# seagochen/unet-segment-pytorch

Hardware: NVIDIA B200
Metric: AttentionUNet 512^2 train images/sec (whole job; per GPU = value / n_gpus) (higher is better)
Workload: dtype bf16

## Files before the change

include/unetb200.h:

```cpp
#ifndef UNETB200_H
#define UNETB200_H
#include <stddef.h>
#include <stdint.h>

#ifdef __cplusplus
extern "C" {
#endif

#define UB2_OK 0
#define UB2_ERR_SHAPE (-1)
#define UB2_ERR_ALIGN (-2)
#define UB2_ERR_WORKSPACE (-3)
#define UB2_ERR_DRIVER (-4)
#define UB2_ERR_ARCH (-5)

int ub2_version(void);
int ub2_num_sms(void);
int ub2_set_conv_mode(int mode);
int ub2_last_conv_variant(void);


int ub2_conv_fwd(const void* in0, int ld_in0, int C0, const void* in1, int ld_in1, int C1,
                 const void* wgt, void* out0, int ld0, void* out1, int ld1, int split, int N, int H,
                 int W, int Cout, int taps, const float* scale, const float* shift, int relu,
                 int accumulate, double* stats, int stats_rows, int* stats_rows_used,
                 int bn_override, int grid_override, void* stream);

int ub2_conv_wgrad(const void* in0, int ld_in0, int C0, const void* in1, int ld_in1, int C1,
                   const void* dy, int ld_dy, float* partial, int max_splits, int* splits_used,
                   int N, int H, int W, int Cout, int taps, int splits_override, void* stream);

int ub2_wgrad_reduce(float* partial, int splits, int Cout, int Cin, int taps, float* grad,
                     int accumulate, void* stream);

#define UB2_REDUCE_MAX_ITEMS 32
typedef struct Ub2ReduceItem {
  float* partial;
  float* grad;
  int splits, Cout, Cin, taps;
} Ub2ReduceItem;
int ub2_wgrad_reduce_multi(const Ub2ReduceItem* items, int n, int accumulate, void* stream);

int ub2_pack_conv_weight(const float* w, void* fwd, void* dgrad, int Cout, int Cin, int taps,
                         const float* out_scale, void* stream);
int ub2_pack_conv_weights_multi(const long long* desc, const int* blocks, int nblocks, void* stream);


int ub2_bn_finalize(const double* partials, int rows, int C, double count, const float* gamma,
                    const float* beta, float* running_mean, float* running_var, long long* nbt,
                    float momentum, float eps, float* scale, float* shift, float* mean, float* invstd,
                    void* stream);
int ub2_bn_eval_coeffs(const float* gamma, const float* beta, const float* running_mean,
                       const float* running_var, float eps, int C, float* scale, float* shift,
                       void* stream);
int ub2_bn_act(const void* y, int ld_y, const float* scale, const float* shift, void* a, int ld_a,
               void* pooled, int ld_p, unsigned char* pidx, int N, int H, int W, int C, int relu,
               void* stream);
int ub2_bn_bwd_rows(int N, int H, int W, int C, int pool);
int ub2_bn_bwd_reduce(const void* dA, int ld_da, const void* dP, int ld_dp, const unsigned char* pidx,
                      const void* y, int ld_y, const float* scale, const float* shift, double* partials,
                      int rows, int N, int H, int W, int C, int relu, void* stream);
int ub2_bn_bwd_finalize(const double* partials, int rows, int C, double count, const float* gamma,
                        const float* mean, const float* invstd, int frozen, float* dgamma, float* dbeta,
                        float* coef, void* stream);
int ub2_bn_bwd_apply(const void* dA, int ld_da, const void* dP, int ld_dp, const unsigned char* pidx,
                     const void* y, int ld_y, const float* scale, const float* shift, const float* coef,
                     void* dY, int ld_dy, int N, int H, int W, int C, int relu, void* stream);


int ub2_upsample_fwd(const void* in, int ld_in, void* out, int ld_out, int N, int hin, int win, int hu,
                     int wu, int Ho, int Wo, int C, void* stream);
int ub2_upsample_bwd(const void* dout, int ld_dout, void* din, int ld_din, int accumulate, int N,
                     int hin, int win, int hu, int wu, int Ho, int Wo, int C, void* stream);

int ub2_shuffle2x2_fwd(const void* t, int ld_t, void* out, int ld_out, int N, int h, int w, int C, int Ho, int Wo,
                       void* stream);
int ub2_shuffle2x2_rows(int N, int h, int w, int C, int Ho, int Wo);
int ub2_shuffle2x2_bwd(const void* dout, int ld_dout, void* dt, int ld_dt, double* partials, int rows, float* dbias,
                       int N, int h, int w, int C, int Ho, int Wo, void* stream);
int ub2_pack_convt_weight(const float* w, const float* bias, void* fwd, void* dg, float* scale4, float* shift4,
                          int Cin, int Cout, void* stream);
int ub2_convt_wgrad_reduce(const float* partial, int splits, int Cin, int Cout, float* grad, int accumulate,
                           void* stream);
int ub2_resize_planes_fwd(const float* in, float* out, int planes, int hin, int win, int Ho, int Wo, void* stream);
int ub2_resize_planes_bwd(const float* dout, float* din, int planes, int hin, int win, int Ho, int Wo,
                          void* stream);


int ub2_gate_rows(int N, int H, int W, int C);
int ub2_gate_strip_rows(int N, int H, int W, int C);
int ub2_gate_upstats(const void* q, int ld_q, int N, int hin, int win, int H, int W, int Ci,
                     double* partials, int rows, void* stream);
int ub2_gate_psi(const void* q, int ld_q, const void* xp, int ld_xp, const float* scale_g,
                 const float* shift_g, const float* scale_x, const float* shift_x, const float* wpsi,
                 float* psi_raw, double* partials, int rows, int N, int hin, int win, int H, int W,
                 int Ci, void* stream);
int ub2_gate_fused_eval(const void* q, int ld_q, const void* xp, int ld_xp, const void* x, int ld_x, const float* scale_g,
                        const float* shift_g, const float* scale_x, const float* shift_x, const float* wpsi,
                        const float* scale_psi, const float* shift_psi, void* out, int ld_out, int N, int hin, int win,
                        int H, int W, int Ci, int Cx, void* stream);
int ub2_gate_apply(const float* psi_raw, const float* scale_psi, const float* shift_psi, const void* x,
                   int ld_x, void* out, int ld_out, float* a_out, int N, int H, int W, int Cx,
                   void* stream);
int ub2_gate_bwd_a(const void* dout, int ld_do, const void* x, int ld_x, const float* a,
                   const float* psi_raw, void* dx, int ld_dx, float* dpsin, double* partials, int rows,
                   int N, int H, int W, int Cx, void* stream);
int ub2_gate_bwd_s(const float* dpsin, const float* psi_raw, const float* coef_psi, const void* q,
                   int ld_q, const void* xp, int ld_xp, const float* scale_g, const float* shift_g,
                   const float* scale_x, const float* shift_x, const float* wpsi, void* ds, int ld_ds,
                   double* partials, int rows, int N, int hin, int win, int H, int W, int Ci,
                   void* stream);
int ub2_gate_bwd_finalize(const double* partials, int rows, int Ci, double count, const float* gamma_x,
                          const float* mean_x, const float* invstd_x, const float* gamma_g,
                          const float* mean_g, const float* invstd_g, int frozen, float* dgamma_x,
                          float* dbeta_x, float* dgamma_g, float* dbeta_g, float* dwpsi, float* coef,
                          void* stream);
int ub2_gate_bwd_xg(const void* ds, int ld_ds, const void* xp, int ld_xp, const void* q, int ld_q,
                    const float* coef, void* dxp, int ld_dxp, void* dgup, int ld_dg, int N, int hin,
                    int win, int H, int W, int Ci, void* stream);


int ub2_conv_in_rows(int N, int H, int W, int Cout);
int ub2_conv_in_fwd(const float* x, const float* w, void* y, int ld_y, double* partials, int rows, int N,
                    int Cin, int H, int W, int Cout, void* stream);
int ub2_conv_in_wgrad(const float* x, const void* dy, int ld_dy, double* partials, int rows, float* grad,
                      int N, int Cin, int H, int W, int Cout, void* stream);
int ub2_conv_in_dgrad(const void* dy, int ld_dy, const float* w, float* dx, int N, int Cin, int H, int W, int Cout,
                      void* stream);
int ub2_outc_rows(int N, int H, int W, int C);
int ub2_outc_fwd(const void* a, int ld_a, const float* w, const float* bias, float* logits, int N, int H,
                 int W, int C, int K, void* stream);
int ub2_outc_bwd(const float* dlogits, const void* a, int ld_a, const float* w, void* da, int ld_da,
                 double* partials, int rows, float* dw, float* db, int N, int H, int W, int C, int K,
                 void* stream);


int ub2_seg_stats_blocks(int N, long long HW);
int ub2_seg_stats(const float* logits, const long long* targets, int N, int C, long long HW,
                  double* partials, int blocks, float* stats, void* stream);
int ub2_seg_stats_bwd(const float* logits, const long long* targets, const float* coef, const float* gscale,
                      int N, int C, long long HW, float* dlogits, void* stream);
int ub2_dice_bce_head(const float* stats, int N, int C, float ce_weight, float dice_weight, float class_weight,
                      float ce_smooth, float dice_smooth, int ignore_background, float* loss, float* coef,
                      void* stream);
int ub2_confusion(const void* pred, const long long* target, int mode, int N, int C, long long HW,
                  long long ignore_index, int has_ignore, float threshold, long long* cm,
                  unsigned char* mask_out, void* stream);


int ub2_conv_fwd_tf32(const float* in0, int ld_in0, int C0, const float* in1, int ld_in1, int C1,
                      const float* wgt, float* out, int ld_out, int N, int H, int W, int Cout, int taps,
                      const float* scale, const float* shift, int relu, int exact_out, void* stream);
int ub2_f32_pack_weight(const float* w, float* out, int Cout, int Cin, int taps, void* stream);
int ub2_f32_conv_in(const float* x, const float* w, const float* scale, const float* shift, float* out, int N,
                    int Cin, int H, int W, int Cout, void* stream);
int ub2_f32_maxpool(const float* in, float* out, int N, int H, int W, int C, void* stream);
int ub2_f32_upsample(const float* in, float* out, int N, int hin, int win, int hu, int wu, int Ho, int Wo, int C,
                     void* stream);
int ub2_f32_gate(const float* q, const float* xp, const float* x, const float* scale_g, const float* shift_g,
                 const float* scale_x, const float* shift_x, const float* w_psi, const float* scale_psi,
                 const float* shift_psi, float* out, int N, int hin, int win, int H, int W, int Ci, int Cx,
                 void* stream);
int ub2_f32_outc(const float* a, const float* w, const float* bias, float* logits, int N, int H, int W, int C,
                 int K, void* stream);


int ub2_adamw_chunk_elems(void);
int ub2_grad_sumsq(const long long* ptrs, const long long* numel, const int* chunks, int nchunks, int T,
                   double* partial, float* step, void* stream);
int ub2_adamw_step(const long long* ptrs, const long long* numel, const int* group, const int* chunks,
                   int nchunks, int T, const double* partial, const float* hyper, const float* step,
                   float* total_norm, int write_grads, void* stream);
int ub2_ema_update(const long long* desc, const int* chunks, int nchunks, const float* decay, void* stream);


int ub2_prepare_batch(const unsigned char* images, const unsigned char* labels, const unsigned char* flags,
                      int N, int H, int W, float mean, float std, float* x, long long* targets,
                      void* stream);
int ub2_predict_mask(const float* logits, int N, int C, long long HW, float threshold, unsigned char* mask,
                     int* positives, void* stream);


int ub2_f32_channel_rows(long long pixels, int C);
int ub2_f32_channel_stats(const float* x, int ld, long long pixels, int C, double* partials, int rows, void* stream);
int ub2_f32_scalar_rows(long long n);
int ub2_f32_scalar_stats(const float* x, long long n, double* partials, int rows, void* stream);
int ub2_f32_affine_act(const float* y, const float* scale, const float* shift, float* out, long long pixels, int C, int relu, void* stream);
int ub2_f32_maxpool_idx(const float* a, float* p, unsigned char* idx, int N, int H, int W, int C, void* stream);
int ub2_f32_act_bwd_reduce(const float* dA, int ld_da, const float* dP, const unsigned char* idx, const float* y, const float* scale, const float* shift, double* partials, int rows, int N, int H, int W, int C, int relu, void* stream);
int ub2_f32_act_bwd_apply(const float* dA, int ld_da, const float* dP, const unsigned char* idx, const float* y, const float* scale, const float* shift, const float* coef, float* dy, int N, int H, int W, int C, int relu, void* stream);
int ub2_f32_upsample_bwd(const float* dout, int ld_dout, float* din, int N, int hin, int win, int hu, int wu, int Ho, int Wo, int C, void* stream);
int ub2_f32_gate_psi(const float* u, const float* xp, const float* sg, const float* hg, const float* sx, const float* hx, const float* wpsi, float* psi_raw, long long pixels, int Ci, void* stream);
int ub2_f32_gate_apply(const float* psi_raw, const float* spsi, const float* hpsi, const float* x, float* out, float* a_out, long long pixels, int Cx, void* stream);
int ub2_f32_gate_rows(long long pixels);
int ub2_f32_gate_bwd_a(const float* dout, int ld_do, const float* x, const float* a, const float* psi_raw, float* dx, float* dpsin, double* partials, int rows, long long pixels, int Cx, void* stream);
int ub2_f32_gate_bwd_s(const float* dpsin, const float* psi_raw, const float* coef_psi, const float* u, const float* xp, const float* sg, const float* hg, const float* sx, const float* hx, const float* wpsi, float* ds, double* partials, int rows, long long pixels, int Ci, void* stream);
int ub2_f32_gate_bwd_xg(const float* ds, const float* xp, const float* u, const float* coef, float* dxp, float* du, long long pixels, int Ci, void* stream);
int ub2_f32_outc_rows(int N, int H, int W);
int ub2_f32_outc_bwd(const float* dlogits, const float* a, const float* w, float* da, double* partials, int rows, float* dw, float* db, int N, int H, int W, int C, int K, void* stream);
int ub2_f32_conv_in_raw(const float* x, const float* w, float* out, int N, int Cin, int H, int W, int Cout, void* stream);
int ub2_f32_conv_in_wgrad(const float* x, const float* dy, double* partials, int rows, float* grad, int N, int Cin, int H, int W, int Cout, void* stream);
int ub2_f32_conv_in_dgrad(const float* dy, int ld_dy, const float* w, float* dx, int N, int Cin, int H, int W, int Cout, void* stream);
int ub2_f32_split_bf16(const float* x, void* hi, void* lo, long long n, void* stream);
int ub2_f32_split_tf32(const float* x0, int ld0, int C0, const float* x1, int ld1, int C1, float* out, long long pixels, void* stream);
int ub2_f32_pack_weight3(const float* w, float* out, int Cout, int Cin, int taps, int dgrad, void* stream);
int ub2_f32_upsample_fwd(const float* in, float* out, int N, int hin, int win, int hu, int wu, int Ho, int Wo, int C, void* stream);
int ub2_f32_shuffle2x2_fwd(const float* t, int ld_t, float* out, int ld_out, int N, int h, int w, int C, int Ho, int Wo, void* stream);
int ub2_f32_shuffle2x2_rows(int N, int h, int w, int C, int Ho, int Wo);
int ub2_f32_shuffle2x2_bwd(const float* dout, int ld_dout, float* dt, int ld_dt, double* partials, int rows, float* dbias, int N, int h, int w, int C, int Ho, int Wo, void* stream);
int ub2_f32_pack_convt_weight(const float* w, const float* bias, float* fwd, float* scale4, float* shift4, int Cin, int Cout, void* stream);

#ifdef __cplusplus
}
#endif
#endif
```

unet-segment-pytorch_b200/csrc/resample.cu:

```cuda
#include "launch.cuh"
#include "../../include/unetb200.h"
#include "conv.h"
#include "resample.cuh"
#include "vec.cuh"

namespace ub2 {

struct UpGeom {
  int N, hin, win, hu, wu, Ho, Wo, pt, pl, C, cgs;
  float rh, rw;
};

__global__ void __launch_bounds__(256)
upsample_fwd_kernel(const __nv_bfloat16* __restrict__ in, int ld_in, __nv_bfloat16* __restrict__ out,
                    int ld_out, UpGeom g) {
  pdl_trigger();
  pdl_wait();
  const int wo = blockIdx.x * blockDim.y + threadIdx.y;
  const int ho = blockIdx.y;
  const int n = blockIdx.z;
  if (wo >= g.Wo) return;
  const int uh = ho - g.pt, uw = wo - g.pl;
  const bool inside = !(uh < 0 || uh >= g.hu || uw < 0 || uw >= g.wu);
  int h0 = 0, h1 = 0, w0 = 0, w1 = 0;
  float a0 = 0.f, a1 = 0.f, b0 = 0.f, b1 = 0.f;
  if (inside) {
    src_index(g.rh, uh, g.hin, h0, h1, a0, a1);
    src_index(g.rw, uw, g.win, w0, w1, b0, b1);
  }
  const __nv_bfloat16* base = in + static_cast<size_t>(n) * g.hin * g.win * ld_in;
  __nv_bfloat16* dst = out + ((static_cast<size_t>(n) * g.Ho + ho) * g.Wo + wo) * ld_out;
  for (int cg = threadIdx.x; cg < g.cgs; cg += blockDim.x) {
    F8 o;
    if (!inside) {
#pragma unroll
      for (int k = 0; k < 8; ++k) o.v[k] = 0.f;
    } else {
      const F8 v00 = load8(base + (static_cast<size_t>(h0) * g.win + w0) * ld_in + cg * 8);
      const F8 v01 = load8(base + (static_cast<size_t>(h0) * g.win + w1) * ld_in + cg * 8);
      const F8 v10 = load8(base + (static_cast<size_t>(h1) * g.win + w0) * ld_in + cg * 8);
      const F8 v11 = load8(base + (static_cast<size_t>(h1) * g.win + w1) * ld_in + cg * 8);
#pragma unroll
      for (int k = 0; k < 8; ++k)
        o.v[k] = a0 * (b0 * v00.v[k] + b1 * v01.v[k]) + a1 * (b0 * v10.v[k] + b1 * v11.v[k]);
    }
    store8(dst + cg * 8, o);
  }
}

static constexpr int kStripRows = 16;

__global__ void __launch_bounds__(256)
upsample_fwd_strip_kernel(const __nv_bfloat16* __restrict__ in, int ld_in, __nv_bfloat16* __restrict__ out,
                          int ld_out, UpGeom g) {
  pdl_trigger();
  pdl_wait();
  const int wo = blockIdx.x * blockDim.y + threadIdx.y;
  const int n = blockIdx.z;
  if (wo >= g.Wo) return;
  const int uw = wo - g.pl;
  const bool col_inside = uw >= 0 && uw < g.wu;
  int w0 = 0, w1 = 0;
  float b0 = 0.f, b1 = 0.f;
  if (col_inside) src_index(g.rw, uw, g.win, w0, w1, b0, b1);
  const __nv_bfloat16* base = in + static_cast<size_t>(n) * g.hin * g.win * ld_in;
  const int ho_begin = blockIdx.y * kStripRows;
  const int ho_end = min(ho_begin + kStripRows, g.Ho);
  for (int cg = threadIdx.x; cg < g.cgs; cg += blockDim.x) {
    auto hrow = [&](int h) {
      const F8 a = load8(base + (static_cast<size_t>(h) * g.win + w0) * ld_in + cg * 8);
      const F8 b = load8(base + (static_cast<size_t>(h) * g.win + w1) * ld_in + cg * 8);
      F8 r;
#pragma unroll
      for (int k = 0; k < 8; ++k) r.v[k] = b0 * a.v[k] + b1 * b.v[k];
      return r;
    };
    int cur0 = -1, cur1 = -1;
    F8 top, bot;
#pragma unroll
    for (int k = 0; k < 8; ++k) top.v[k] = bot.v[k] = 0.f;
    for (int ho = ho_begin; ho < ho_end; ++ho) {
      const int uh = ho - g.pt;
      F8 o;
#pragma unroll
      for (int k = 0; k < 8; ++k) o.v[k] = 0.f;
      if (col_inside && uh >= 0 && uh < g.hu) {
        int h0, h1;
        float a0, a1;
        src_index(g.rh, uh, g.hin, h0, h1, a0, a1);
        if (h0 != cur0) {
          top = (h0 == cur1) ? bot : hrow(h0);
          cur0 = h0;
        }
        if (h1 != cur1) {
          bot = (h1 == cur0) ? top : hrow(h1);
          cur1 = h1;
        }
#pragma unroll
        for (int k = 0; k < 8; ++k) o.v[k] = a0 * top.v[k] + a1 * bot.v[k];
      }
      store8(out + ((static_cast<size_t>(n) * g.Ho + ho) * g.Wo + wo) * ld_out + cg * 8, o);
    }
  }
}

__device__ __forceinline__ float tap_weight(float r, int u, int in, int i) {
  int i0, i1;
  float l0, l1;
  src_index(r, u, in, i0, i1, l0, l1);
  float w = 0.f;
  if (i0 == i) w += l0;
  if (i1 == i) w += l1;
  return w;
}

__device__ __forceinline__ void dst_range(float r, int i, int out, int& lo, int& hi) {
  if (r <= 0.f) {
    lo = 0;
    hi = out - 1;
    return;
  }
  lo = static_cast<int>(floorf((static_cast<float>(i) - 1.f) / r)) - 1;
  hi = static_cast<int>(ceilf((static_cast<float>(i) + 1.f) / r)) + 1;
  if (lo < 0) lo = 0;
  if (hi > out - 1) hi = out - 1;
}

static constexpr int kMaxTaps = 8;

__global__ void __launch_bounds__(256)
upsample_bwd_kernel(const __nv_bfloat16* __restrict__ dout, int ld_dout,
                    __nv_bfloat16* __restrict__ din, int ld_din, int accumulate, UpGeom g) {
  pdl_trigger();
  pdl_wait();
  const int wi = blockIdx.x * blockDim.y + threadIdx.y;
  const int hi = blockIdx.y;
  const int n = blockIdx.z;
  if (wi >= g.win) return;
  int ulo, uhi, vlo, vhi;
  dst_range(g.rh, hi, g.hu, ulo, uhi);
  dst_range(g.rw, wi, g.wu, vlo, vhi);
  int vs[kMaxTaps];
  float wv[kMaxTaps];
  int nv = 0;
  bool overflow = false;
  for (int v = vlo; v <= vhi; ++v) {
    const float ww = tap_weight(g.rw, v, g.win, wi);
    const int wo = v + g.pl;
    if (ww == 0.f || wo < 0 || wo >= g.Wo) continue;
    if (nv < kMaxTaps) {
#pragma unroll
      for (int k = 0; k < kMaxTaps; ++k)
        if (k == nv) { vs[k] = wo; wv[k] = ww; }
      ++nv;
    } else {
      overflow = true;
    }
  }
  __nv_bfloat16* dst = din + ((static_cast<size_t>(n) * g.hin + hi) * g.win + wi) * ld_din;
  for (int cg = threadIdx.x; cg < g.cgs; cg += blockDim.x) {
    F8 acc;
#pragma unroll
    for (int k = 0; k < 8; ++k) acc.v[k] = 0.f;
    for (int u = ulo; u <= uhi; ++u) {
      const float wh = tap_weight(g.rh, u, g.hin, hi);
      const int ho = u + g.pt;
      if (wh == 0.f || ho < 0 || ho >= g.Ho) continue;
      const __nv_bfloat16* row = dout + (static_cast<size_t>(n) * g.Ho + ho) * g.Wo * ld_dout + cg * 8;
      if (!overflow) {
#pragma unroll
        for (int k = 0; k < kMaxTaps; ++k) {
          if (k < nv) {
            const F8 d = load8(row + static_cast<size_t>(vs[k]) * ld_dout);
            const float wt = wh * wv[k];
#pragma unroll
            for (int c = 0; c < 8; ++c) acc.v[c] = fmaf(wt, d.v[c], acc.v[c]);
          }
        }
      } else {
        for (int v = vlo; v <= vhi; ++v) {
          const float ww = tap_weight(g.rw, v, g.win, wi);
          const int wo = v + g.pl;
          if (ww == 0.f || wo < 0 || wo >= g.Wo) continue;
          const F8 d = load8(row + static_cast<size_t>(wo) * ld_dout);
          const float wt = wh * ww;
#pragma unroll
          for (int c = 0; c < 8; ++c) acc.v[c] = fmaf(wt, d.v[c], acc.v[c]);
        }
      }
    }
    if (accumulate) {
      const F8 old = load8(dst + cg * 8);
#pragma unroll
      for (int k = 0; k < 8; ++k) acc.v[k] += old.v[k];
    }
    store8(dst + cg * 8, acc);
  }
}

static constexpr int kBT_H = 8, kBT_W = 16;
static constexpr int kBT_RH = 24, kBT_RW = 40;

__global__ void __launch_bounds__(256)
upsample_bwd_tiled_kernel(const __nv_bfloat16* __restrict__ dout, int ld_dout,
                          __nv_bfloat16* __restrict__ din, int ld_din, int accumulate, int slabs, UpGeom g) {
  pdl_trigger();
  pdl_wait();
  __shared__ uint4 region[kBT_RH * kBT_RW * 2];
  const int slab = blockIdx.z % slabs;
  const int n = blockIdx.z / slabs;
  const int h0 = blockIdx.y * kBT_H, w0 = blockIdx.x * kBT_W;
  const int h_last = min(h0 + kBT_H, g.hin) - 1, w_last = min(w0 + kBT_W, g.win) - 1;
  int ulo, uhi, vlo, vhi, t0, t1;
  dst_range(g.rh, h0, g.hu, ulo, t0);
  dst_range(g.rh, h_last, g.hu, t1, uhi);
  dst_range(g.rw, w0, g.wu, vlo, t0);
  dst_range(g.rw, w_last, g.wu, t1, vhi);
  const int RW = vhi - vlo + 1, RH = uhi - ulo + 1;
  const int tid = threadIdx.x;
  const __nv_bfloat16* src = dout + static_cast<size_t>(n) * g.Ho * g.Wo * ld_dout + slab * 16;
  constexpr int kLoads = (kBT_RH * kBT_RW * 2 + 255) / 256;
  uint4 stage[kLoads];
#pragma unroll
  for (int k = 0; k < kLoads; ++k) {
    const int idx = tid + k * 256;
    const int col = (idx >> 1) % kBT_RW;
    const int row = (idx >> 1) / kBT_RW;
    const int ho = ulo + row + g.pt, wo = vlo + col + g.pl;
    stage[k] = make_uint4(0u, 0u, 0u, 0u);
    if (row < RH && col < RW && ho >= 0 && ho < g.Ho && wo >= 0 && wo < g.Wo)
      stage[k] = __ldg(reinterpret_cast<const uint4*>(src + (static_cast<size_t>(ho) * g.Wo + wo) * ld_dout) + (idx & 1));
  }
#pragma unroll
  for (int k = 0; k < kLoads; ++k) {
    const int idx = tid + k * 256;
    if (idx < kBT_RH * kBT_RW * 2) region[idx] = stage[k];
  }
  __syncthreads();
  const int half = tid & 1;
  const int wi = w0 + ((tid >> 1) & (kBT_W - 1));
  const int hi = h0 + (tid >> 5);
  if (wi >= g.win || hi >= g.hin) return;
  const float fi = static_cast<float>(hi), fj = static_cast<float>(wi);
  int u0 = static_cast<int>(floorf((fi - 1.f) / g.rh)) + 1;
  int v0 = static_cast<int>(floorf((fj - 1.f) / g.rw)) + 1;
  if (u0 < 0) u0 = 0;
  if (v0 < 0) v0 = 0;
  float wv[5];
  int cv[5];
#pragma unroll
  for (int k = 0; k < 5; ++k) {
    const int v = v0 + k;
    wv[k] = (v < g.wu) ? fmaxf(0.f, 1.f - fabsf(g.rw * static_cast<float>(v) - fj)) : 0.f;
    cv[k] = (min(v, vhi) - vlo) * 2;
  }
  F8 acc;
#pragma unroll
  for (int k = 0; k < 8; ++k) acc.v[k] = 0.f;
#pragma unroll
  for (int kr = 0; kr < 5; ++kr) {
    const int u = u0 + kr;
    const float wh = (u < g.hu) ? fmaxf(0.f, 1.f - fabsf(g.rh * static_cast<float>(u) - fi)) : 0.f;
    if (wh == 0.f) continue;
    const uint4* rowp = region + (min(u, uhi) - ulo) * (kBT_RW * 2) + half;
#pragma unroll
    for (int k = 0; k < 5; ++k) {
      const F8 d = unpack8(rowp[cv[k]]);
      const float wt = wh * wv[k];
#pragma unroll
      for (int c = 0; c < 8; ++c) acc.v[c] = fmaf(wt, d.v[c], acc.v[c]);
    }
  }
  __nv_bfloat16* dst = din + ((static_cast<size_t>(n) * g.hin + hi) * g.win + wi) * ld_din + slab * 16 + half * 8;
  if (accumulate) {
    const F8 old = load8(dst);
#pragma unroll
    for (int k = 0; k < 8; ++k) acc.v[k] += old.v[k];
  }
  store8(dst, acc);
}

static bool bwd_tiled_ok(const UpGeom& g) {
  if (g.C % 16 != 0 || g.rh <= 0.f || g.rw <= 0.f) return false;
  const float span_h = (static_cast<float>(kBT_H) + 1.f) / g.rh + 5.f;
  const float span_w = (static_cast<float>(kBT_W) + 1.f) / g.rw + 5.f;
  return span_h <= kBT_RH && span_w <= kBT_RW && g.rw >= 0.4f && g.rh >= 0.4f;
}

static constexpr int kBwdStrip = 16;

__global__ void __launch_bounds__(256)
upsample_bwd_strip_kernel(const __nv_bfloat16* __restrict__ dout, int ld_dout, __nv_bfloat16* __restrict__ din,
                          int ld_din, int accumulate, int strip, UpGeom g) {
  pdl_trigger();
  pdl_wait();
  const int j = blockIdx.x * blockDim.y + threadIdx.y;
  const int n = blockIdx.z;
  if (j >= g.win) return;
  const int ia = blockIdx.y * strip, ib = min(ia + strip, g.hin);
  const float fj = static_cast<float>(j);
  int v0 = static_cast<int>(floorf((fj - 1.f) / g.rw)) + 1;
  if (v0 < 0) v0 = 0;
  float wv[5];
  int cv[5];
#pragma unroll
  for (int k = 0; k < 5; ++k) {
    const int v = v0 + k;
    wv[k] = (v < g.wu) ? fmaxf(0.f, 1.f - fabsf(g.rw * static_cast<float>(v) - fj)) : 0.f;
    cv[k] = min(v, g.wu - 1) + g.pl;
  }
  int u_lo = static_cast<int>(floorf(static_cast<float>(ia - 1) / g.rh)) - 1;
  int u_hi = static_cast<int>(ceilf(static_cast<float>(ib) / g.rh)) + 1;
  if (u_lo < 0) u_lo = 0;
  if (u_hi > g.hu - 1) u_hi = g.hu - 1;
  const __nv_bfloat16* src = dout + static_cast<size_t>(n) * g.Ho * g.Wo * ld_dout;
  __nv_bfloat16* dst = din + (static_cast<size_t>(n) * g.hin * g.win + j) * ld_din;
  for (int cg = threadIdx.x; cg < g.cgs; cg += blockDim.x) {
    auto flush = [&](int row, const F8& acc) {
      if (row < ia || row >= ib) return;
      __nv_bfloat16* q = dst + static_cast<size_t>(row) * g.win * ld_din + cg * 8;
      F8 o = acc;
      if (accumulate) {
        const F8 old = load8(q);
#pragma unroll
        for (int k = 0; k < 8; ++k) o.v[k] += old.v[k];
      }
      store8(q, o);
    };
    F8 acc0, acc1;
#pragma unroll
    for (int k = 0; k < 8; ++k) acc0.v[k] = acc1.v[k] = 0.f;
    int r_cur = -2;
    for (int u = u_lo; u <= u_hi; ++u) {
      int i0, i1;
      float l0, l1;
      src_index(g.rh, u, g.hin, i0, i1, l0, l1);
      if (i0 < ia - 1 || i0 > ib - 1) continue;
      if (r_cur == -2) r_cur = i0;
      while (i0 > r_cur) {
        flush(r_cur, acc0);
        acc0 = acc1;
#pragma unroll
        for (int k = 0; k < 8; ++k) acc1.v[k] = 0.f;
        ++r_cur;
      }
      const __nv_bfloat16* rowp = src + static_cast<size_t>(u + g.pt) * g.Wo * ld_dout + cg * 8;
      F8 t;
#pragma unroll
      for (int k = 0; k < 8; ++k) t.v[k] = 0.f;
#pragma unroll
      for (int k = 0; k < 5; ++k) {
        if (wv[k] != 0.f) {
          const F8 d = load8(rowp + static_cast<size_t>(cv[k]) * ld_dout);
#pragma unroll
          for (int c = 0; c < 8; ++c) t.v[c] = fmaf(wv[k], d.v[c], t.v[c]);
        }
      }
      if (i1 == i0) {
#pragma unroll
        for (int k = 0; k < 8; ++k) acc0.v[k] = fmaf(l0 + l1, t.v[k], acc0.v[k]);
      } else {
#pragma unroll
        for (int k = 0; k < 8; ++k) {
          acc0.v[k] = fmaf(l0, t.v[k], acc0.v[k]);
          acc1.v[k] = fmaf(l1, t.v[k], acc1.v[k]);
        }
      }
    }
    if (r_cur != -2) {
      flush(r_cur, acc0);
      flush(r_cur + 1, acc1);
    }
  }
}

static bool bwd_strip_ok(const UpGeom& g) {
  return g.rh >= 0.4f && g.rh <= 0.6f && g.rw >= 0.4f && g.rw <= 0.6f && g.hin >= 2 * kBwdStrip;
}

static dim3 up_block(int cgs) {
  int bx = 1;
  while (bx < cgs && bx < 256) bx *= 2;
  return dim3(bx, 256 / bx);
}

static UpGeom up_geom(int N, int hin, int win, int hu, int wu, int Ho, int Wo, int C) {
  UpGeom g;
  g.N = N; g.hin = hin; g.win = win; g.hu = hu; g.wu = wu; g.Ho = Ho; g.Wo = Wo; g.C = C;
  g.cgs = C / 8;
  g.pt = (Ho - hu) / 2;
  g.pl = (Wo - wu) / 2;
  g.rh = hu > 1 ? static_cast<float>(hin - 1) / static_cast<float>(hu - 1) : 0.f;
  g.rw = wu > 1 ? static_cast<float>(win - 1) / static_cast<float>(wu - 1) : 0.f;
  return g;
}

__global__ void __launch_bounds__(256)
resize_planes_fwd_kernel(const float* __restrict__ in, float* __restrict__ out, int planes, LowRes g) {
  pdl_trigger();
  pdl_wait();
  const long long total = static_cast<long long>(planes) * g.Ho * g.Wo;
  for (long long idx = static_cast<long long>(blockIdx.x) * blockDim.x + threadIdx.x; idx < total;
       idx += static_cast<long long>(gridDim.x) * blockDim.x) {
    const int wo = static_cast<int>(idx % g.Wo);
    const long long row = idx / g.Wo;
    const int ho = static_cast<int>(row % g.Ho);
    const long long p = row / g.Ho;
    int h0, h1, w0, w1;
    float a0, a1, b0, b1;
    src_index(g.rh, ho, g.hin, h0, h1, a0, a1);
    src_index(g.rw, wo, g.win, w0, w1, b0, b1);
    const float* base = in + p * g.hin * g.win;
    const float v00 = __ldg(base + h0 * g.win + w0), v01 = __ldg(base + h0 * g.win + w1);
    const float v10 = __ldg(base + h1 * g.win + w0), v11 = __ldg(base + h1 * g.win + w1);
    out[idx] = a0 * (b0 * v00 + b1 * v01) + a1 * (b0 * v10 + b1 * v11);
  }
}

__global__ void __launch_bounds__(256)
resize_planes_bwd_kernel(const float* __restrict__ dout, float* __restrict__ din, int planes, LowRes g) {
  pdl_trigger();
  pdl_wait();
  const long long total = static_cast<long long>(planes) * g.hin * g.win;
  for (long long idx = static_cast<long long>(blockIdx.x) * blockDim.x + threadIdx.x; idx < total;
       idx += static_cast<long long>(gridDim.x) * blockDim.x) {
    const int j = static_cast<int>(idx % g.win);
    const long long row = idx / g.win;
    const int i = static_cast<int>(row % g.hin);
    const long long p = row / g.hin;
    int ylo, yhi, xlo, xhi;
    dst_range(g.rh, i, g.Ho, ylo, yhi);
    dst_range(g.rw, j, g.Wo, xlo, xhi);
    const float* base = dout + p * g.Ho * g.Wo;
    float acc = 0.f;
    for (int y = ylo; y <= yhi; ++y) {
      const float wy = tap_weight(g.rh, y, g.hin, i);
      if (wy == 0.f) continue;
      float rowacc = 0.f;
      for (int x = xlo; x <= xhi; ++x) {
        const float wx = tap_weight(g.rw, x, g.win, j);
        if (wx != 0.f) rowacc = fmaf(wx, __ldg(base + static_cast<long long>(y) * g.Wo + x), rowacc);
      }
      acc = fmaf(wy, rowacc, acc);
    }
    din[idx] = acc;
  }
}

}

using namespace ub2;

extern "C" {

int ub2_upsample_fwd(const void* in, int ld_in, void* out, int ld_out, int N, int hin, int win, int hu,
                     int wu, int Ho, int Wo, int C, void* stream) {
  if (C <= 0 || C % 8 != 0 || Ho < hu || Wo < wu || N <= 0 || hin <= 0 || win <= 0 || hu <= 0 || wu <= 0)
    return UB2_ERR_SHAPE;
  if (ld_in % 8 || ld_out % 8) return UB2_ERR_ALIGN;
  UpGeom g = up_geom(N, hin, win, hu, wu, Ho, Wo, C);
  if (Ho >= 2 * kStripRows) {
    const dim3 sblock = up_block(g.cgs);
    const dim3 sgrid((Wo + sblock.y - 1) / sblock.y, (Ho + kStripRows - 1) / kStripRows, N);
    launch(upsample_fwd_strip_kernel, sgrid, sblock, 0, static_cast<cudaStream_t>(stream), static_cast<const __nv_bfloat16*>(in), ld_in, static_cast<__nv_bfloat16*>(out), ld_out, g);
    return static_cast<int>(cudaGetLastError());
  }
  const dim3 block = up_block(g.cgs);
  const dim3 grid((Wo + block.y - 1) / block.y, Ho, N);
  launch(upsample_fwd_kernel, grid, block, 0, static_cast<cudaStream_t>(stream), static_cast<const __nv_bfloat16*>(in), ld_in, static_cast<__nv_bfloat16*>(out), ld_out, g);
  return static_cast<int>(cudaGetLastError());
}

int ub2_upsample_bwd(const void* dout, int ld_dout, void* din, int ld_din, int accumulate, int N,
                     int hin, int win, int hu, int wu, int Ho, int Wo, int C, void* stream) {
  if (C <= 0 || C % 8 != 0 || Ho < hu || Wo < wu || N <= 0 || hin <= 0 || win <= 0 || hu <= 0 || wu <= 0)
    return UB2_ERR_SHAPE;
  if (ld_dout % 8 || ld_din % 8) return UB2_ERR_ALIGN;
  UpGeom g = up_geom(N, hin, win, hu, wu, Ho, Wo, C);
  if (bwd_strip_ok(g)) {
    const dim3 sblock = up_block(g.cgs);
    const long long wave = static_cast<long long>(num_sms()) * 2048;
    int strip = kBwdStrip;
    while (strip > 2 && static_cast<long long>(N) * ((hin + strip - 1) / strip) * win * g.cgs < wave) strip >>= 1;
    const dim3 sgrid((win + sblock.y - 1) / sblock.y, (hin + strip - 1) / strip, N);
    launch(upsample_bwd_strip_kernel, sgrid, sblock, 0, static_cast<cudaStream_t>(stream), static_cast<const __nv_bfloat16*>(dout), ld_dout, static_cast<__nv_bfloat16*>(din), ld_din, accumulate, strip, g);
    return static_cast<int>(cudaGetLastError());
  }
  if (bwd_tiled_ok(g)) {
    const int slabs = C / 16;
    const dim3 tgrid((win + kBT_W - 1) / kBT_W, (hin + kBT_H - 1) / kBT_H, N * slabs);
    launch(upsample_bwd_tiled_kernel, tgrid, 256, 0, static_cast<cudaStream_t>(stream), static_cast<const __nv_bfloat16*>(dout), ld_dout, static_cast<__nv_bfloat16*>(din), ld_din, accumulate, slabs, g);
    return static_cast<int>(cudaGetLastError());
  }
  const dim3 block = up_block(g.cgs);
  const dim3 grid((win + block.y - 1) / block.y, hin, N);
  launch(upsample_bwd_kernel, grid, block, 0, static_cast<cudaStream_t>(stream), static_cast<const __nv_bfloat16*>(dout), ld_dout, static_cast<__nv_bfloat16*>(din), ld_din, accumulate, g);
  return static_cast<int>(cudaGetLastError());
}

int ub2_resize_planes_fwd(const float* in, float* out, int planes, int hin, int win, int Ho, int Wo, void* stream) {
  if (planes <= 0 || hin <= 0 || win <= 0 || Ho <= 0 || Wo <= 0) return UB2_ERR_SHAPE;
  const long long total = static_cast<long long>(planes) * Ho * Wo;
  launch(resize_planes_fwd_kernel, stream_grid(total, 256, num_sms(), 8), 256, 0, static_cast<cudaStream_t>(stream), in, out, planes, make_lowres(hin, win, Ho, Wo));
  return static_cast<int>(cudaGetLastError());
}

int ub2_resize_planes_bwd(const float* dout, float* din, int planes, int hin, int win, int Ho, int Wo,
                          void* stream) {
  if (planes <= 0 || hin <= 0 || win <= 0 || Ho <= 0 || Wo <= 0) return UB2_ERR_SHAPE;
  const long long total = static_cast<long long>(planes) * hin * win;
  launch(resize_planes_bwd_kernel, stream_grid(total, 256, num_sms(), 8), 256, 0, static_cast<cudaStream_t>(stream), dout, din, planes, make_lowres(hin, win, Ho, Wo));
  return static_cast<int>(cudaGetLastError());
}

}
```

Measured before the change: 592.8.

## Add shared-memory tiled bilinear upsample backward kernel with cp.async staging

Adds a new backward kernel for the 2x bilinear upsample gradient. Each block stages a 2D tile of the output gradient into shared memory with cp.async, using a swizzled column layout, and then computes a tile of input-gradient pixels from it. This replaces the strip kernel as the default when the strip conditions hold, aiming to cut redundant global reads of overlapping taps. It also adds variant tracking and an environment switch back to the old path. The cost is a large dynamic shared-memory allocation that may limit occupancy.

```diff
diff --git a/include/unetb200.h b/include/unetb200.h
--- a/include/unetb200.h
+++ b/include/unetb200.h
@@ -72,6 +72,13 @@
                      int wu, int Ho, int Wo, int C, void* stream);
 int ub2_upsample_bwd(const void* dout, int ld_dout, void* din, int ld_din, int accumulate, int N,
                      int hin, int win, int hu, int wu, int Ho, int Wo, int C, void* stream);
+#define UB2_UPSAMPLE_FWD_PIXEL 1
+#define UB2_UPSAMPLE_FWD_STRIP 2
+#define UB2_UPSAMPLE_BWD_DIRECT 11
+#define UB2_UPSAMPLE_BWD_TILED 12
+#define UB2_UPSAMPLE_BWD_STRIP 13
+#define UB2_UPSAMPLE_BWD_TILE 14
+int ub2_last_upsample_variant(void);
 
 int ub2_shuffle2x2_fwd(const void* t, int ld_t, void* out, int ld_out, int N, int h, int w, int C, int Ho, int Wo,
                        void* stream);
diff --git a/unet-segment-pytorch_b200/csrc/resample.cu b/unet-segment-pytorch_b200/csrc/resample.cu
--- a/unet-segment-pytorch_b200/csrc/resample.cu
+++ b/unet-segment-pytorch_b200/csrc/resample.cu
@@ -10,6 +10,10 @@
   int N, hin, win, hu, wu, Ho, Wo, pt, pl, C, cgs;
   float rh, rw;
 };
+
+__device__ __forceinline__ float hat_weight(float r, int v, int out, float fj) {
+  return (v < out) ? fmaxf(0.f, 1.f - fabsf(r * static_cast<float>(v) - fj)) : 0.f;
+}
 
 __global__ void __launch_bounds__(256)
 upsample_fwd_kernel(const __nv_bfloat16* __restrict__ in, int ld_in, __nv_bfloat16* __restrict__ out,
@@ -306,7 +310,7 @@
 #pragma unroll
   for (int k = 0; k < 5; ++k) {
     const int v = v0 + k;
-    wv[k] = (v < g.wu) ? fmaxf(0.f, 1.f - fabsf(g.rw * static_cast<float>(v) - fj)) : 0.f;
+    wv[k] = hat_weight(g.rw, v, g.wu, fj);
     cv[k] = min(v, g.wu - 1) + g.pl;
   }
   int u_lo = static_cast<int>(floorf(static_cast<float>(ia - 1) / g.rh)) - 1;
@@ -378,11 +382,167 @@
   return g.rh >= 0.4f && g.rh <= 0.6f && g.rw >= 0.4f && g.rw <= 0.6f && g.hin >= 2 * kBwdStrip;
 }
 
+#ifndef UB2_TI
+#define UB2_TI 8
+#define UB2_TJ 16
+#define UB2_TC 4
+#define UB2_TR 4
+#endif
+static constexpr int kTI = UB2_TI, kTJ = UB2_TJ, kTC = UB2_TC, kTR = UB2_TR;
+static constexpr int kTileThreads = kTJ * kTC * (kTI / kTR);
+
+__device__ __forceinline__ int tile_col(int c) { return c ^ ((c >> 1) & 1); }
+
+__device__ __forceinline__ void cp_async16(void* smem, const void* gmem) {
+  asm volatile("cp.async.cg.shared.global [%0], [%1], 16;" ::"r"(static_cast<uint32_t>(__cvta_generic_to_shared(smem))),
+               "l"(gmem)
+               : "memory");
+}
+
+__global__ void __launch_bounds__(kTileThreads)
+upsample_bwd_tile_kernel(const __nv_bfloat16* __restrict__ dout, int ld_dout, __nv_bfloat16* __restrict__ din,
+                         int ld_din, int accumulate, int slabs, int tile_pitch, UpGeom g) {
+  extern __shared__ uint4 tile[];
+  pdl_trigger();
+  pdl_wait();
+  const int slab = blockIdx.x % slabs;
+  const int ja = (blockIdx.x / slabs) * kTJ, jb = min(ja + kTJ, g.win);
+  const int ia = blockIdx.y * kTI, ib = min(ia + kTI, g.hin);
+  const int n = blockIdx.z;
+  const int cg0 = slab * kTC, nc = min(kTC, g.cgs - cg0);
+  int u_lo = static_cast<int>(floorf(static_cast<float>(ia - 1) / g.rh)) - 1;
+  int u_hi = static_cast<int>(ceilf(static_cast<float>(ib) / g.rh)) + 1;
+  if (u_lo < 0) u_lo = 0;
+  if (u_hi > g.hu - 1) u_hi = g.hu - 1;
+  int u_first = -1, u_last = -2;
+  for (int u = u_lo; u <= u_hi; ++u) {
+    int i0, i1;
+    float l0, l1;
+    src_index(g.rh, u, g.hin, i0, i1, l0, l1);
+    if (i0 >= ia - 1 && i0 <= ib - 1) {
+      if (u_first < 0) u_first = u;
+      u_last = u;
+    }
+  }
+  auto first_tap = [&](int j) {
+    const int v = static_cast<int>(floorf((static_cast<float>(j) - 1.f) / g.rw)) + 1;
+    return v < 0 ? 0 : v;
+  };
+  const int v_first = first_tap(ja);
+  const int v_last = min(first_tap(jb - 1) + 4, g.wu - 1);
+  const int rows = u_last - u_first + 1, cols = v_last - v_first + 1;
+  const int lane = threadIdx.x & 31;
+  const __nv_bfloat16* src = dout + static_cast<size_t>(n) * g.Ho * g.Wo * ld_dout + cg0 * 8;
+  for (int r = threadIdx.x >> 5; r < rows; r += kTileThreads / 32) {
+    const __nv_bfloat16* srow = src + static_cast<size_t>(u_first + r + g.pt) * g.Wo * ld_dout;
+    uint4* trow = tile + r * tile_pitch;
+    for (int e = lane; e < cols * kTC; e += 32) {
+      const int c = e / kTC, q = e % kTC;
+      if (q < nc) cp_async16(trow + tile_col(c) * kTC + q, srow + static_cast<size_t>(v_first + c + g.pl) * ld_dout + q * 8);
+    }
+  }
+  asm volatile("cp.async.wait_all;" ::: "memory");
+  __syncthreads();
+
+  const int q = threadIdx.x % kTC;
+  const int j = ja + (threadIdx.x / kTC) % kTJ;
+  const int ra = ia + (threadIdx.x / (kTC * kTJ)) * kTR;
+  const int rb = min(ra + kTR, ib);
+  if (j >= jb || q >= nc || ra >= rb) return;
+  const float fj = static_cast<float>(j);
+  int v0 = static_cast<int>(floorf((fj - 1.f) / g.rw)) + 1;
+  if (v0 < 0) v0 = 0;
+  float wv[5];
+  int cv[5];
+#pragma unroll
+  for (int k = 0; k < 5; ++k) {
+    const int v = v0 + k;
+    wv[k] = hat_weight(g.rw, v, g.wu, fj);
+    cv[k] = tile_col(min(v, g.wu - 1) - v_first) * kTC + q;
+  }
+  __nv_bfloat16* dst = din + (static_cast<size_t>(n) * g.hin * g.win + j) * ld_din + (cg0 + q) * 8;
+  auto flush = [&](int row, const F8& acc) {
+    if (row < ra || row >= rb) return;
+    __nv_bfloat16* p = dst + static_cast<size_t>(row) * g.win * ld_din;
+    F8 o = acc;
+    if (accumulate) {
+      const F8 old = load8(p);
+#pragma unroll
+      for (int k = 0; k < 8; ++k) o.v[k] += old.v[k];
+    }
+    store8(p, o);
+  };
+  F8 acc0, acc1;
+#pragma unroll
+  for (int k = 0; k < 8; ++k) acc0.v[k] = acc1.v[k] = 0.f;
+  int r_cur = -2;
+  for (int u = u_first; u <= u_last; ++u) {
+    int i0, i1;
+    float l0, l1;
+    src_index(g.rh, u, g.hin, i0, i1, l0, l1);
+    if (i0 < ra - 1 || i0 > rb - 1) continue;
+    if (r_cur == -2) r_cur = i0;
+    while (i0 > r_cur) {
+      flush(r_cur, acc0);
+      acc0 = acc1;
+#pragma unroll
+      for (int k = 0; k < 8; ++k) acc1.v[k] = 0.f;
+      ++r_cur;
+    }
+    const uint4* rowp = tile + (u - u_first) * tile_pitch;
+    F8 t;
+#pragma unroll
+    for (int k = 0; k < 8; ++k) t.v[k] = 0.f;
+#pragma unroll
+    for (int k = 0; k < 5; ++k) {
+      if (wv[k] != 0.f) {
+        const F8 d = unpack8(rowp[cv[k]]);
+#pragma unroll
+        for (int c = 0; c < 8; ++c) t.v[c] = fmaf(wv[k], d.v[c], t.v[c]);
+      }
+    }
+    if (i1 == i0) {
+#pragma unroll
+      for (int k = 0; k < 8; ++k) acc0.v[k] = fmaf(l0 + l1, t.v[k], acc0.v[k]);
+    } else {
+#pragma unroll
+      for (int k = 0; k < 8; ++k) {
+        acc0.v[k] = fmaf(l0, t.v[k], acc0.v[k]);
+        acc1.v[k] = fmaf(l1, t.v[k], acc1.v[k]);
+      }
+    }
+  }
+  if (r_cur != -2) {
+    flush(r_cur, acc0);
+    flush(r_cur + 1, acc1);
+  }
+}
+
+static int bwd_tile_pitch(const UpGeom& g) {
+  int cols = static_cast<int>(static_cast<float>(kTJ - 1) / g.rw) + 7;
+  cols += cols & 1;
+  return cols * kTC;
+}
+static size_t bwd_tile_smem(const UpGeom& g) {
+  const int rows = static_cast<int>(static_cast<float>(kTI + 1) / g.rh) + 3;
+  return static_cast<size_t>(rows) * bwd_tile_pitch(g) * sizeof(uint4);
+}
+
 static dim3 up_block(int cgs) {
   int bx = 1;
   while (bx < cgs && bx < 256) bx *= 2;
   return dim3(bx, 256 / bx);
 }
+
+static bool upsample_legacy() {
+  static const bool on = [] {
+    const char* e = getenv("UB2_UPSAMPLE_LEGACY");
+    return e != nullptr && atoi(e) != 0;
+  }();
+  return on;
+}
+
+static thread_local int g_up_variant = 0;
 
 static UpGeom up_geom(int N, int hin, int win, int hu, int wu, int Ho, int Wo, int C) {
   UpGeom g;
@@ -462,11 +622,13 @@
   if (Ho >= 2 * kStripRows) {
     const dim3 sblock = up_block(g.cgs);
     const dim3 sgrid((Wo + sblock.y - 1) / sblock.y, (Ho + kStripRows - 1) / kStripRows, N);
+    g_up_variant = UB2_UPSAMPLE_FWD_STRIP;
     launch(upsample_fwd_strip_kernel, sgrid, sblock, 0, static_cast<cudaStream_t>(stream), static_cast<const __nv_bfloat16*>(in), ld_in, static_cast<__nv_bfloat16*>(out), ld_out, g);
     return static_cast<int>(cudaGetLastError());
   }
   const dim3 block = up_block(g.cgs);
   const dim3 grid((Wo + block.y - 1) / block.y, Ho, N);
+  g_up_variant = UB2_UPSAMPLE_FWD_PIXEL;
   launch(upsample_fwd_kernel, grid, block, 0, static_cast<cudaStream_t>(stream), static_cast<const __nv_bfloat16*>(in), ld_in, static_cast<__nv_bfloat16*>(out), ld_out, g);
   return static_cast<int>(cudaGetLastError());
 }
@@ -477,26 +639,46 @@
     return UB2_ERR_SHAPE;
   if (ld_dout % 8 || ld_din % 8) return UB2_ERR_ALIGN;
   UpGeom g = up_geom(N, hin, win, hu, wu, Ho, Wo, C);
+  if (bwd_strip_ok(g) && !upsample_legacy()) {
+    static PerDevice<bool> attr_set_pd;
+    bool& attr_set = attr_set_pd.ref();
+    if (!attr_set) {
+      const cudaError_t e = cudaFuncSetAttribute(upsample_bwd_tile_kernel, cudaFuncAttributeMaxDynamicSharedMemorySize,
+                                                 227 * 1024);
+      if (e != cudaSuccess) return static_cast<int>(e);
+      attr_set = true;
+    }
+    const int slabs = (g.cgs + kTC - 1) / kTC;
+    const dim3 tgrid(((win + kTJ - 1) / kTJ) * slabs, (hin + kTI - 1) / kTI, N);
+    g_up_variant = UB2_UPSAMPLE_BWD_TILE;
+    launch(upsample_bwd_tile_kernel, tgrid, kTileThreads, bwd_tile_smem(g), static_cast<cudaStream_t>(stream), static_cast<const __nv_bfloat16*>(dout), ld_dout, static_cast<__nv_bfloat16*>(din), ld_din, accumulate, slabs, bwd_tile_pitch(g), g);
+    return static_cast<int>(cudaGetLastError());
+  }
   if (bwd_strip_ok(g)) {
     const dim3 sblock = up_block(g.cgs);
     const long long wave = static_cast<long long>(num_sms()) * 2048;
     int strip = kBwdStrip;
     while (strip > 2 && static_cast<long long>(N) * ((hin + strip - 1) / strip) * win * g.cgs < wave) strip >>= 1;
     const dim3 sgrid((win + sblock.y - 1) / sblock.y, (hin + strip - 1) / strip, N);
+    g_up_variant = UB2_UPSAMPLE_BWD_STRIP;
     launch(upsample_bwd_strip_kernel, sgrid, sblock, 0, static_cast<cudaStream_t>(stream), static_cast<const __nv_bfloat16*>(dout), ld_dout, static_cast<__nv_bfloat16*>(din), ld_din, accumulate, strip, g);
     return static_cast<int>(cudaGetLastError());
   }
   if (bwd_tiled_ok(g)) {
     const int slabs = C / 16;
     const dim3 tgrid((win + kBT_W - 1) / kBT_W, (hin + kBT_H - 1) / kBT_H, N * slabs);
+    g_up_variant = UB2_UPSAMPLE_BWD_TILED;
     launch(upsample_bwd_tiled_kernel, tgrid, 256, 0, static_cast<cudaStream_t>(stream), static_cast<const __nv_bfloat16*>(dout), ld_dout, static_cast<__nv_bfloat16*>(din), ld_din, accumulate, slabs, g);
     return static_cast<int>(cudaGetLastError());
   }
   const dim3 block = up_block(g.cgs);
   const dim3 grid((win + block.y - 1) / block.y, hin, N);
+  g_up_variant = UB2_UPSAMPLE_BWD_DIRECT;
   launch(upsample_bwd_kernel, grid, block, 0, static_cast<cudaStream_t>(stream), static_cast<const __nv_bfloat16*>(dout), ld_dout, static_cast<__nv_bfloat16*>(din), ld_din, accumulate, g);
   return static_cast<int>(cudaGetLastError());
 }
+
+int ub2_last_upsample_variant(void) { return g_up_variant; }
 
 int ub2_resize_planes_fwd(const float* in, float* out, int planes, int hin, int win, int Ho, int Wo, void* stream) {
   if (planes <= 0 || hin <= 0 || win <= 0 || Ho <= 0 || Wo <= 0) return UB2_ERR_SHAPE;
```

Result: no change. 588.3, median of 6 (-0.8%).
